# Wionerlol/MultimodalEmotionRecognition

Hardware: AMD Instinct MI355X
Metric: 3s-clip train steps/sec (B=32, xattn fusion) at 1/2/4/8 MI355X (higher is better)
Workload: dtype bf16; 1 GPU; ResNet18 + WavLM-base (frozen) + xattn fusion train step (fwd+bwd+Adam); per_gpu_batch=32, global_batch=32, frames=8, image=112, audio_samples=48000, parallelism=dp1

## Files before the change

### multimodalemotionrecognition_amd/csrc/conv.hip

```cpp
#include <type_traits>

#include "common.h"
#include "mer.h"

typedef __attribute__((ext_vector_type(4))) uint32_t u32x4;
typedef __attribute__((ext_vector_type(4))) short s16x4;

#ifdef MER_CONV_TIMING
static __device__ long long mer_ct_buf[512 * 64];
#define CT(k) \
  do { \
    if (threadIdx.x == 0 && blockIdx.x < 512 && (k) < 64) mer_ct_buf[blockIdx.x * 64 + (k)] = wall_clock64(); \
  } while (0)
MER_API int mer_ct_reset() {
  static long long zeros[512 * 64];
  return (int)hipMemcpyToSymbol(HIP_SYMBOL(mer_ct_buf), zeros, sizeof(zeros), 0, hipMemcpyHostToDevice);
}
MER_API int mer_ct_read(long long* host) {
  return (int)hipMemcpyFromSymbol(host, HIP_SYMBOL(mer_ct_buf), sizeof(long long) * 512 * 64, 0, hipMemcpyDeviceToHost);
}
static __device__ long long mer_ctp_buf[4096 * 8];
#define CTP(k) \
  do { \
    const unsigned b_ = blockIdx.y * gridDim.x + blockIdx.x; \
// ... 297 lines not shown
    for (int j = 0; j < JT; ++j) acc[i][j] = f32x4{0.f, 0.f, 0.f, 0.f};

  const int nk = (p_end - p_beg + 63) / 64;
  auto compute = [&](int cur) {
    const bf16_t* Aimg = &lds[cur][0];
    const bf16_t* Bimg = &lds[cur][64 * LDM];
#pragma unroll
    for (int s = 0; s < 2; ++s) {
      bf16x8 af[IT], bfr[JT];
#pragma unroll
      for (int i = 0; i < IT; ++i) af[i] = tr_frag(Aimg, LDM, s * 32, wm + i * 16);
#pragma unroll
      for (int j = 0; j < JT; ++j) bfr[j] = tr_frag(Bimg, LDN, s * 32, wn + j * 16);
#pragma unroll
      for (int i = 0; i < IT; ++i)
#pragma unroll
        for (int j = 0; j < JT; ++j) acc[i][j] = __builtin_amdgcn_mfma_f32_16x16x32_bf16(af[i], bfr[j], acc[i][j], 0, 0, 0);
    }
  };
  if (PF == 1) {
    if (nk > 0) {
      gload(ra, rb, okm, p_beg);
      lstore(0, ra, rb, okm);
    }
    __syncthreads();
    for (int kt = 0; kt < nk; ++kt) {
      const int cur = kt & 1;
      gload(ra, rb, okm, p_beg + (kt + 1 < nk ? kt + 1 : kt) * 64);
      compute(cur);
      if (kt + 1 < nk) lstore(cur ^ 1, ra, rb, okm);
      __syncthreads();
    }
  } else {
    auto kstep = [&](int k) { return p_beg + (k < nk ? k : nk - 1) * 64; };
    if (nk > 0) {
      gload(ra, rb, okm, p_beg);
      gload(ra2, rb2, okm2, kstep(1));
      lstore(0, ra, rb, okm);
    }
    lds_barrier();
    for (int kt = 0; kt < nk; kt += 2) {
      gload(ra, rb, okm, kstep(kt + 2));
      compute(0);
      if (kt + 1 < nk) lstore(1, ra2, rb2, okm2);
      lds_barrier();
      if (kt + 1 >= nk) break;
      gload(ra2, rb2, okm2, kstep(kt + 3));
      compute(1);
      if (kt + 2 < nk) lstore(0, ra, rb, okm);
      lds_barrier();
    }
  }
  float* slab = g.ws + (long)blockIdx.z * g.K * Ntot;
#pragma unroll
  for (int i = 0; i < IT; ++i)
#pragma unroll
    for (int j = 0; j < JT; ++j) {
      const int nn = n0 + wn + j * 16 + (lane & 15);
      if (nn >= Ntot) continue;
#pragma unroll
      for (int rr = 0; rr < 4; ++rr) {
        const int k = m0 + wm + i * 16 + (lane >> 4) * 4 + rr;
        if (k < g.K) slab[(long)k * Ntot + nn] = acc[i][j][rr];
      }
    }
}

__device__ __attribute__((aligned(16))) uint32_t mer_conv_zero16[4] = {0u, 0u, 0u, 0u};

__device__ __forceinline__ int wswz(int row, int nchunks) { return ((row & 7) << 1) & (nchunks - 1); }

template <int BM_, int BN_, int WM, int WN, int STAGES, int KS = 64, int KG = 1>
__global__ __launch_bounds__(64 * WM * WN * KG, KG > 1 ? WM * WN * KG / 4 : 2) void wgrad_pipe_kernel(WgradGeom g) {
  constexpr int WAVES = WM * WN;
  constexpr int ACW = BM_ / 8, BCW = BN_ / 8;
  constexpr int ARI = 64 / ACW, BRI = 64 / BCW;
  constexpr int IA = KS / ARI / WAVES, IB = KS / BRI / WAVES;
  static_assert(IA * ARI * WAVES == KS && IB * BRI * WAVES == KS, "the K-step must split into whole glds rows");
  static_assert(KS % 32 == 0, "MFMA k = 32 pixels");
  constexpr int IT = BM_ / WM / 16, JT = BN_ / WN / 16;
  constexpr int BUF = KS * (BM_ + BN_);
  extern __shared__ __attribute__((aligned(16))) bf16_t smem_all[];
  const int t = threadIdx.x, lane = t & 63, kg = (t >> 6) / WAVES, w = (t >> 6) % WAVES;
  bf16_t* const smem = smem_all + kg * STAGES * BUF;
  const int Ntot = g.R * g.S * g.C;
  const int P = g.N * g.Ho * g.Wo;
  const int wnx = (Ntot + BN_ - 1) / BN_, wny = (g.K + BM_ - 1) / BM_;
  int wtx, wty, zs;
  if (g.flat) {
    int tile;
    xcd_tile(blockIdx.x, wnx * wny, (int)gridDim.x, tile, zs);
    wty = tile / wnx;
    wtx = tile - wty * wnx;
  } else {
    xcd_tile(blockIdx.x, wnx, wnx * wny, wtx, wty);
    zs = blockIdx.z;
  }
  const int m0 = wty * BM_, n0 = wtx * BN_;
  const int p_beg = zs * g.pix_per_split, p_end = min(P, p_beg + g.pix_per_split);
  const int wm = (w / WN) * (BM_ / WM), wn = (w % WN) * (BN_ / WN);
  const bf16_t* zero = reinterpret_cast<const bf16_t*>(mer_conv_zero16);

  int arow[IA], acol[IA];
  bool acok[IA];
#pragma unroll
  for (int j = 0; j < IA; ++j) {
    const int row = (w * IA + j) * ARI + lane / ACW;
    arow[j] = row;
    acol[j] = m0 + ((lane % ACW) ^ wswz(row, ACW)) * 8;
    acok[j] = acol[j] < g.K;
  }
  int brow[IB], bc[IB], br[IB], bs[IB];
  bool bcok[IB];
  const float inv_C = 1.f / g.C, inv_S = 1.f / g.S, inv_HoWo = 1.f / (g.Ho * g.Wo), inv_Wo = 1.f / g.Wo;
#pragma unroll
  for (int j = 0; j < IB; ++j) {
    const int row = (w * IB + j) * BRI + lane / BCW;
    brow[j] = row;
    const int col = n0 + ((lane % BCW) ^ wswz(row, BCW)) * 8;
    bcok[j] = col < Ntot;
    const int cc = bcok[j] ? col : 0;
    const int tap = fdiv(cc, inv_C);
    bc[j] = cc - tap * g.C;
    br[j] = fdiv(tap, inv_S);
    bs[j] = tap - br[j] * g.S;
  }
  const int HoWo = g.Ho * g.Wo;
  auto stage = [&](int slot, int p0) {
    bf16_t* la = smem + slot * BUF;
    bf16_t* lb = la + KS * BM_;
#pragma unroll
    for (int j = 0; j < IA; ++j) {
      const int p = p0 + arow[j];
      glds16(p < p_end && acok[j] ? g.dY + (long)p * g.ldy + acol[j] : zero, la + (w * IA + j) * 512);
    }
#pragma unroll
    for (int j = 0; j < IB; ++j) {
      const int p = p0 + brow[j];
      const int pc = p < p_end ? p : p_beg;
      const int n = fdiv(pc, inv_HoWo);
      const int rem = pc - n * HoWo;
      const int oh = fdiv(rem, inv_Wo), ow = rem - oh * g.Wo;
      const int ih = oh * g.st - g.pad + br[j], iw = ow * g.st - g.pad + bs[j];
      const bool ok = p < p_end && bcok[j] && ih >= 0 && ih < g.H && iw >= 0 && iw < g.W;
      glds16(ok ? g.X + (((long)n * g.H + ih) * g.W + iw) * g.C + bc[j] : zero, lb + (w * IB + j) * 512);
    }
  };
  auto tr_frag = [&](const bf16_t* img, int CW, int k0, int c0) -> bf16x8 {
    const int q = (lane & 15) >> 2, p4 = (lane & 3) * 4;
    const int kr = k0 + 8 * (lane >> 4);
    const int lc = (c0 + p4) >> 3, sub = (c0 + p4) & 7;
    typedef __attribute__((address_space(3))) s16x4 lds_s16x4;
    const int r0 = kr + q, r1 = kr + 4 + q;
    const s16x4 lo = __builtin_amdgcn_ds_read_tr16_b64_v4i16(
        (lds_s16x4*)(img + r0 * CW * 8 + ((lc ^ wswz(r0, CW)) << 3) + sub));
    const s16x4 hi = __builtin_amdgcn_ds_read_tr16_b64_v4i16(
        (lds_s16x4*)(img + r1 * CW * 8 + ((lc ^ wswz(r1, CW)) << 3) + sub));
    typedef __attribute__((ext_vector_type(8))) short s16x8;
    s16x8 v = {lo[0], lo[1], lo[2], lo[3], hi[0], hi[1], hi[2], hi[3]};
    return __builtin_bit_cast(bf16x8, v);
  };

  f32x4 acc[IT][JT];
#pragma unroll
  for (int i = 0; i < IT; ++i)
#pragma unroll
    for (int j = 0; j < JT; ++j) acc[i][j] = f32x4{0.f, 0.f, 0.f, 0.f};
  const int nk_all = (p_end - p_beg + KS - 1) / KS;
  const int nkg = (nk_all + KG - 1) / KG, kb = kg * nkg;
  const int nk = nk_all - kb < nkg ? (nk_all - kb > 0 ? nk_all - kb : 0) : nkg;
  const int pk0 = p_beg + kb * KS;
  constexpr int G = IA + IB;
#pragma unroll
  for (int s = 0; s < STAGES - 1; ++s)
    if (s < nk) stage(s, pk0 + s * KS);
  for (int kt = 0; kt < nkg; ++kt) {
    const int left = nk - 1 - kt;
    const int ahead = left < (STAGES - 2) ? left : (STAGES - 2);
    wait_tiles_in_flight<G>(ahead);
    lds_barrier();
    if (kt + STAGES - 1 < nk) stage((kt + STAGES - 1) % STAGES, pk0 + (kt + STAGES - 1) * KS);
    if (KG > 1 && kt >= nk) continue;
    const bf16_t* Aimg = smem + (kt % STAGES) * BUF;
    const bf16_t* Bimg = Aimg + KS * BM_;
#pragma unroll
    for (int s = 0; s < KS / 32; ++s) {
      bf16x8 af[IT], bfr[JT];
#pragma unroll
      for (int i = 0; i < IT; ++i) af[i] = tr_frag(Aimg, ACW, s * 32, wm + i * 16);
#pragma unroll
      for (int j = 0; j < JT; ++j) bfr[j] = tr_frag(Bimg, BCW, s * 32, wn + j * 16);
      __builtin_amdgcn_s_setprio(1);
#pragma unroll
      for (int i = 0; i < IT; ++i)
#pragma unroll
        for (int j = 0; j < JT; ++j) acc[i][j] = __builtin_amdgcn_mfma_f32_16x16x32_bf16(af[i], bfr[j], acc[i][j], 0, 0, 0);
      __builtin_amdgcn_s_setprio(0);
    }
  }
  if constexpr (KG > 1) {
    constexpr int LDR = BN_ + 4;
    __syncthreads();
    float* const part = reinterpret_cast<float*>(smem_all);
    if (kg > 0) {
      float* mine = part + (kg - 1) * BM_ * LDR;
#pragma unroll
      for (int i = 0; i < IT; ++i)
#pragma unroll
        for (int j = 0; j < JT; ++j)
#pragma unroll
          for (int rr = 0; rr < 4; ++rr)
            mine[(wm + i * 16 + (lane >> 4) * 4 + rr) * LDR + wn + j * 16 + (lane & 15)] = acc[i][j][rr];
    }
    lds_barrier();
    if (kg > 0) return;
#pragma unroll
    for (int i = 0; i < IT; ++i)
#pragma unroll
      for (int j = 0; j < JT; ++j)
#pragma unroll
        for (int rr = 0; rr < 4; ++rr)
#pragma unroll
          for (int q = 1; q < KG; ++q)
            acc[i][j][rr] += part[(q - 1) * BM_ * LDR + (wm + i * 16 + (lane >> 4) * 4 + rr) * LDR + wn + j * 16 +
                                  (lane & 15)];
  }
  float* slab = g.ws + (long)zs * g.K * Ntot;
#pragma unroll
  for (int i = 0; i < IT; ++i)
#pragma unroll
    for (int j = 0; j < JT; ++j) {
      const int nn = n0 + wn + j * 16 + (lane & 15);
      if (nn >= Ntot) continue;
#pragma unroll
      for (int rr = 0; rr < 4; ++rr) {
        const int k = m0 + wm + i * 16 + (lane >> 4) * 4 + rr;
        if (k < g.K) slab[(long)k * Ntot + nn] = acc[i][j][rr];
      }
    }
}

template <int BM_, int BN_, int WM, int WN, int STAGES, int KS = 64, int KG = 1>
void launch_wgrad_pipe(const WgradGeom& g0, dim3 grid, hipStream_t st) {
  const size_t ring = (size_t)KG * STAGES * KS * (BM_ + BN_) * sizeof(bf16_t);
  const size_t xchg = (size_t)(KG - 1) * BM_ * (BN_ + 4) * sizeof(float);
  const size_t lds = ring > xchg ? ring : xchg;
  if (hipFuncSetAttribute(reinterpret_cast<const void*>(&wgrad_pipe_kernel<BM_, BN_, WM, WN, STAGES, KS, KG>),
                          hipFuncAttributeMaxDynamicSharedMemorySize, (int)lds) != hipSuccess)
    return;
  WgradGeom g = g0;
  g.flat = 1;
  const dim3 gr(grid.x * grid.z, 1, 1);
  hipLaunchKernelGGL((wgrad_pipe_kernel<BM_, BN_, WM, WN, STAGES, KS, KG>), gr, dim3(64 * WM * WN * KG), lds, st, g);
}

__global__ __launch_bounds__(256) void wgrad_reduce_kernel(int K, int C, int Creal, int RS, int splits, int SG,
                                                           float* __restrict__ ws) {
  __shared__ float part[256];
  const int E = 256 / SG, e = threadIdx.x % E, sg = threadIdx.x / E;
  const long total = (long)K * RS * C;
  const long idx = (long)blockIdx.x * E + e;
  float a0 = 0.f, a1 = 0.f, a2 = 0.f, a3 = 0.f;
  if (idx < total) {
    int z = sg;
    for (; z + 3 * SG < splits; z += 4 * SG) {
      a0 += ws[(long)z * total + idx];
      a1 += ws[(long)(z + SG) * total + idx];
      a2 += ws[(long)(z + 2 * SG) * total + idx];
      a3 += ws[(long)(z + 3 * SG) * total + idx];
    }
    for (; z < splits; z += SG) a0 += ws[(long)z * total + idx];
  }
  part[threadIdx.x] = (a0 + a1) + (a2 + a3);
  __syncthreads();
  if (sg != 0 || idx >= total) return;
  float s = 0.f;
  for (int q = 0; q < SG; ++q) s += part[q * E + e];
  ws[idx] = s;
}

__global__ __launch_bounds__(256) void wgrad_fold_scatter_kernel(int K, int C, int Creal, int RS, int splits,
                                                                 const float* __restrict__ ws, float* __restrict__ dw) {
  __shared__ float tile[49 * 32];
  const int k = blockIdx.y, c0 = blockIdx.x * 32;
  const long slab = (long)K * RS * C;
  const float* src = ws + (long)k * RS * C;
  for (int i = threadIdx.x; i < RS * 32; i += 256) {
    const int tap = i >> 5, c = c0 + (i & 31);
    const float* e = src + tap * C + (c < Creal ? c : 0);
    float s = 0.f;
    for (int z0 = 0; z0 < splits; z0 += 8) {
      float v[8];
#pragma unroll
      for (int q = 0; q < 8; ++q) v[q] = e[(long)(z0 + q < splits ? z0 + q : splits - 1) * slab];
#pragma unroll
      for (int q = 0; q < 8; ++q) s += z0 + q < splits ? v[q] : 0.f;
    }
    tile[i] = c < Creal ? s : 0.f;
  }
  __syncthreads();
  const int ncl = min(32, Creal - c0);
  const float inv_RS = 1.f / RS;
  float* dst = dw + ((long)k * Creal + c0) * RS;
  for (int i = threadIdx.x; i < ncl * RS; i += 256) {
    const int cl = fdiv(i, inv_RS), tap = i - cl * RS;
    dst[i] += tile[tap * 32 + cl];
  }
}

__global__ __launch_bounds__(256) void wgrad_scatter_kernel(int C, int Creal, int RS, const float* __restrict__ ws,
                                                            float* __restrict__ dw) {
  __shared__ float tile[49 * 32];
  const int k = blockIdx.y, c0 = blockIdx.x * 32;
  const float* src = ws + (long)k * RS * C;
  for (int i = threadIdx.x; i < RS * 32; i += 256) {
    const int tap = i >> 5, c = c0 + (i & 31);
    tile[i] = c < Creal ? src[tap * C + c] : 0.f;
  }
  __syncthreads();
  const int ncl = min(32, Creal - c0);
  const float inv_RS = 1.f / RS;
  float* dst = dw + ((long)k * Creal + c0) * RS;
// ... 480 lines not shown
    }
    flush();
    return;
  }
  conv_tile_stats<FM, FN, WM, WN>(g, acc, smemf, w, lane, m0, n0, M, stat_row);
  if (ct_slot >= 0) CT(ct_slot + 1);
  flush();
  if (ct_slot >= 0) CT(ct_slot + 2);
}

template <bool DGRAD, int FM, int FN, int WM, int WN, int WAVE_FLOATS, bool X2 = true>
__device__ __forceinline__ void conv_epilogue_acc_finish(const ConvGeom& g, EpiAcc<FN>& a, float* smemf, int w,
                                                         int lane, int n0, long row_id) {
  if constexpr (DGRAD) {
    if (!g.bnr_red) return;
    using E = EpiGeo<FM, FN, WAVE_FLOATS>;
    constexpr int TN = FN * 16, LPR = E::LPR;
    const int wr = w / WN, wc = w % WN;
    const int lc = (lane % LPR) * 8;
    const int colv = n0 + wc * TN + lc;
    const bool cok = colv < g.Ncols;
    const bool has_x2 = X2 && g.bnr_x2 != nullptr;
#pragma unroll
    for (int o = LPR; o < 64; o <<= 1)
#pragma unroll
      for (int e = 0; e < 8; ++e) {
        a.sA[e] += __shfl_xor(a.sA[e], o, 64);
        a.sB[e] += __shfl_xor(a.sB[e], o, 64);
        if (has_x2) a.sC[e] += __shfl_xor(a.sC[e], o, 64);
      }
    float* red = smemf;
    lds_barrier();
    if (wr > 0 && lane < LPR)
#pragma unroll
      for (int e = 0; e < 8; ++e) {
        float* o = red + ((wr * WN + wc) * TN + lc + e) * 3;
        o[0] = a.sA[e];
        o[1] = a.sB[e];
        o[2] = a.sC[e];
      }
    lds_barrier();
    if (wr != 0 || lane >= LPR || !cok) return;
#pragma unroll
    for (int e = 0; e < 8; ++e)
#pragma unroll
      for (int q = 1; q < WM; ++q) {
        const float* o = red + ((q * WN + wc) * TN + lc + e) * 3;
        a.sA[e] += o[0];
        a.sB[e] += o[1];
        a.sC[e] += o[2];
      }
    const long slab = row_id * g.Ncols * 2 + 2 * colv;
#pragma unroll
    for (int e = 0; e < 8; e += 2) {
      *reinterpret_cast<f32x4*>(g.bnr_red + slab + 2 * e) = f32x4{a.sA[e], a.sB[e], a.sA[e + 1], a.sB[e + 1]};
      if (g.bnr_red2)
        *reinterpret_cast<f32x4*>(g.bnr_red2 + slab + 2 * e) = f32x4{a.sA[e], a.sC[e], a.sA[e + 1], a.sC[e + 1]};
    }
  } else {
    if (!g.stats) return;
    conv_stats_finish<FN, WM, WN>(g, a.fs, smemf, w, lane, n0, row_id);
  }
}

constexpr int conv_pipe_wpe(int nw, int bm, int bn, int stages, bool dgrad, bool par, int lds_bytes = 0) {
  return (nw >= 16 || 2 * lds_bytes > 160 * 1024)
             ? (nw >= 4 ? nw / 4 : 1)
             : nw == 8 ? ((dgrad && (bm == 256 || (!par && bm == 128 && bn == 128 && stages == 3))) ? 2 : 4) : 2;
}
constexpr int conv_pipe_lds(int bm, int bn, int stages, int ks, int kg) {
  return kg * stages * (bm + bn) * ks * 2 > (kg > 1 ? kg * bm * (bn + 4) * 4 : 0)
             ? kg * stages * (bm + bn) * ks * 2
             : kg * bm * (bn + 4) * 4;
}

template <int BM_, int BN_, int NW>
struct KgLayout {
  static constexpr int WM = (NW >= 4 && BM_ / 4 >= 16) ? 4 : (NW >= 2 ? 2 : 1);
  static constexpr int WN = NW / WM;
  static_assert(WM * WN == NW && BM_ % (16 * WM) == 0 && BN_ % (16 * WN) == 0, "split-K epilogue layout");
};

template <bool DGRAD, bool PAR, int BM_, int BN_, int WM = 2, int WN = 2, int STAGES = 2, int KS = 64, bool X2 = true,
          int KG = 1>
__global__ __launch_bounds__(64 * WM * WN * KG, conv_pipe_wpe(WM * WN * KG, BM_, BN_, STAGES, DGRAD, PAR,
                                                              conv_pipe_lds(BM_, BN_, STAGES, KS, KG))) void conv_pipe_kernel(ConvGeom g) {
  constexpr int WAVES = WM * WN;
  constexpr int CW = KS / 8, RPG = 64 / CW;
  constexpr int IA = BM_ / RPG / WAVES, IB = BN_ / RPG / WAVES;
  static_assert(IA * RPG * WAVES == BM_ && IB * RPG * WAVES == BN_, "tile rows must split into whole glds pieces");
  static_assert(KS == 64 || KS == 32, "K-tile");
  static_assert(KG == 1 || KG == 2 || KG == 4, "K-groups");
  constexpr int TM = BM_ / WM, TN = BN_ / WN, FM = TM / 16, FN = TN / 16;
  constexpr int BUF = (BM_ + BN_) * KS;
  extern __shared__ __attribute__((aligned(16))) bf16_t smem_all[];
  const int t = threadIdx.x, lane = t & 63, kg = (t >> 6) / WAVES, w = (t >> 6) % WAVES;
  bf16_t* const smem = smem_all + kg * STAGES * BUF;
  ParClass pc{};
  int M, Kr, rowsH, rowsW;
  int Kr0 = 0;
  if (PAR) {
    pc = par_class(g, par_cls());
    M = g.N * pc.Hc * pc.Wc;
    Kr0 = pc.nr * pc.ns * g.IC;
    Kr = Kr0 + ((g.X2 && pc.ph == 0 && pc.pw == 0) ? g.K2 : 0);
    rowsH = pc.Hc;
    rowsW = pc.Wc;
  } else {
    M = g.N * g.OH * g.OW;
    Kr = g.Kred;
    rowsH = g.OH;
    rowsW = g.OW;
  }
  const int nx = (g.Ncols + BN_ - 1) / BN_, ny = (M + BM_ - 1) / BM_;
  if ((int)blockIdx.x >= nx * ny) return;
  CTP(0);
  int tx, ty;
  xcd_tile(blockIdx.x, nx, nx * ny, tx, ty);
  const int m0 = ty * BM_, n0 = tx * BN_;
  const int wr = w / WN, wc = w % WN;

  int an[IA], aoh[IA], aow[IA], acl[IA];
  bool aok[IA];
#pragma unroll
  for (int j = 0; j < IA; ++j) {
    const int r = (w * IA + j) * RPG + lane / CW;
    const int m = m0 + r;
    aok[j] = m < M;
    const int mm = aok[j] ? m : 0;
    an[j] = mm / (rowsH * rowsW);
    const int rem = mm - an[j] * rowsH * rowsW;
    aoh[j] = rem / rowsW;
    aow[j] = rem - aoh[j] * rowsW;
    acl[j] = cswz_k<CW>(r, lane % CW) * 8;
  }
  const bf16_t* pb[IB];
  const bf16_t* pb2[IB];
  int bcl[IB];
  bool bok[IB];
#pragma unroll
  for (int j = 0; j < IB; ++j) {
    const int r = (w * IB + j) * RPG + lane / CW;
    const int n = n0 + r;
    bok[j] = n < g.Ncols;
    pb[j] = g.Wt + (long)(bok[j] ? n : 0) * g.Kred;
    pb2[j] = g.Wt2 + (long)(bok[j] ? n : 0) * g.K2;
    bcl[j] = cswz_k<CW>(r, lane % CW) * 8;
  }
  const float inv_IC = 1.f / g.IC, inv_S = 1.f / g.S, inv_ns = PAR ? 1.f / pc.ns : 1.f;
  const bf16_t* zero = reinterpret_cast<const bf16_t*>(mer_conv_zero16);
  auto par_a_src = [&](int n, int hh, int ww, bool rowok, int kk) -> const bf16_t* {
    if (!rowok || kk >= Kr) return zero;
    if (kk >= Kr0)
      return g.X2 + (((long)n * g.IH + hh) * g.IW + ww) * g.K2 + (kk - Kr0);
    const int tap = fdiv(kk, inv_IC), c = kk - tap * g.IC;
    const int ri = fdiv(tap, inv_ns), si = tap - ri * pc.ns;
    const int ih = hh + pc.dh0 - ri, iw = ww + pc.dw0 - si;
    if (ih < 0 || ih >= g.IH || iw < 0 || iw >= g.IW) return zero;
    return g.X + (((long)n * g.IH + ih) * g.IW + iw) * g.IC + c;
  };
  auto par_b_off = [&](int kk) -> int {
    const int tap = fdiv(kk, inv_IC), c = kk - tap * g.IC;
    const int ri = fdiv(tap, inv_ns), si = tap - ri * pc.ns;
    return ((pc.r0 + 2 * ri) * g.S + pc.s0 + 2 * si) * g.IC + c;
  };
  auto stage = [&](int buf, int k0) {
    bf16_t* la = smem + buf * BUF;
    bf16_t* lb = la + BM_ * KS;
#pragma unroll
    for (int j = 0; j < IA; ++j) {
      const bf16_t* src = PAR ? par_a_src(an[j], aoh[j], aow[j], aok[j], k0 + acl[j])
                              : conv_a_src<DGRAD>(g, an[j], aoh[j], aow[j], aok[j], k0 + acl[j], inv_IC, inv_S);
      glds16(src, la + (w * IA + j) * 512);
    }
#pragma unroll
    for (int j = 0; j < IB; ++j) {
      const int kk = k0 + bcl[j];
      const bool ok = bok[j] && kk < Kr;
      const bf16_t* src = !PAR ? pb[j] + kk : (kk >= Kr0 ? pb2[j] + (kk - Kr0) : pb[j] + par_b_off(kk));
      glds16(ok ? src : zero, lb + (w * IB + j) * 512);
    }
  };

  f32x4 acc[FM][FN];
#pragma unroll
  for (int i = 0; i < FM; ++i)
#pragma unroll
    for (int j = 0; j < FN; ++j) acc[i][j] = f32x4{0.f, 0.f, 0.f, 0.f};

  const int fr = lane & 15, fq = lane >> 4;
  const int nk_all = (Kr + KS - 1) / KS;
  const int nkg = (nk_all + KG - 1) / KG, kb = kg * nkg;
  const int nk = nk_all - kb < nkg ? (nk_all - kb > 0 ? nk_all - kb : 0) : nkg;
  const int kofs = kb * KS;
  constexpr int G = IA + IB;
  static_assert(STAGES >= 2 && STAGES <= 4, "ring depth");
#pragma unroll
  for (int p = 0; p < STAGES - 1; ++p)
    if (p < nk) stage(p, kofs + p * KS);
  CTP(1);
  for (int kt = 0; kt < nkg; ++kt) {
    const int left = nk - 1 - kt;
    const int ahead = left < (STAGES - 2) ? left : (STAGES - 2);
    wait_tiles_in_flight<G>(ahead);
    lds_barrier();
    if (kt + STAGES - 1 < nk) stage((kt + STAGES - 1) % STAGES, kofs + (kt + STAGES - 1) * KS);
    if (KG > 1 && kt >= nk) continue;
    const bf16_t* la = smem + (kt % STAGES) * BUF;
    const bf16_t* lb = la + BM_ * KS;
#pragma unroll
    for (int s = 0; s < KS / 32; ++s) {
      bf16x8 af[FM], bfr[FN];
#pragma unroll
      for (int i = 0; i < FM; ++i) {
        const int r = wr * TM + i * 16 + fr;
        af[i] = *reinterpret_cast<const bf16x8*>(la + r * KS + cswz_k<CW>(r, s * 4 + fq) * 8);
      }
#pragma unroll
      for (int j = 0; j < FN; ++j) {
        const int r = wc * TN + j * 16 + fr;
        bfr[j] = *reinterpret_cast<const bf16x8*>(lb + r * KS + cswz_k<CW>(r, s * 4 + fq) * 8);
      }
      __builtin_amdgcn_s_setprio(1);
#pragma unroll
      for (int i = 0; i < FM; ++i)
#pragma unroll
        for (int j = 0; j < FN; ++j) acc[i][j] = __builtin_amdgcn_mfma_f32_16x16x32_bf16(af[i], bfr[j], acc[i][j], 0, 0, 0);
      __builtin_amdgcn_s_setprio(0);
    }
  }
  CTP(2);

  auto out_row = [&](int row) -> long {
    if (!PAR) return (long)row;
    const int n = row / (pc.Hc * pc.Wc);
    const int rem = row - n * pc.Hc * pc.Wc;
    const int hh = rem / pc.Wc, ww = rem - hh * pc.Wc;
    return ((long)n * g.OH + 2 * hh + pc.ph) * g.OW + 2 * ww + pc.pw;
  };
  auto red_row = [&]() -> long {
    long row_id = ty;
    if (PAR)
      for (int c2 = 0; c2 < par_cls(); ++c2) {
        const ParClass q = par_class(g, c2);
        row_id += (g.N * q.Hc * q.Wc + BM_ - 1) / BM_;
      }
    return row_id;
  };
  constexpr int EWF = STAGES * BUF / 2 / WAVES;
  const int ct_slot = 10;
  if constexpr (KG > 1) {
    using L = KgLayout<BM_, BN_, WAVES * KG>;
    constexpr int LDR = BN_ + 4;
    constexpr int TM2 = BM_ / L::WM, TN2 = BN_ / L::WN, FM2 = TM2 / 16, FN2 = TN2 / 16;
    using E2 = EpiGeo<FM2, FN2, EWF>;
    const int w2 = t >> 6, wr2 = w2 / L::WN, wc2 = w2 % L::WN;
    constexpr bool PF = DGRAD && E2::NP == 1;
    EpiPre<E2::NP> pre;
    if constexpr (PF)
      conv_epilogue_prefetch<DGRAD, FM2, FN2, L::WM, L::WN, EWF, decltype(out_row), E2::NP, X2>(g, pre, w2, lane, m0,
                                                                                                n0, M, out_row);
    __syncthreads();
    float* const part = reinterpret_cast<float*>(smem_all);
    {
      float* mine = part + kg * BM_ * LDR;
#pragma unroll
      for (int i = 0; i < FM; ++i)
#pragma unroll
        for (int j = 0; j < FN; ++j)
#pragma unroll
          for (int r = 0; r < 4; ++r) mine[(wr * TM + i * 16 + fq * 4 + r) * LDR + wc * TN + j * 16 + fr] = acc[i][j][r];
    }
    lds_barrier();
    f32x4 acc2[FM2][FN2];
#pragma unroll
    for (int i = 0; i < FM2; ++i)
#pragma unroll
      for (int j = 0; j < FN2; ++j)
#pragma unroll
        for (int r = 0; r < 4; ++r) {
          const int e = (wr2 * TM2 + i * 16 + fq * 4 + r) * LDR + wc2 * TN2 + j * 16 + fr;
          float s = part[e];
#pragma unroll
          for (int q = 1; q < KG; ++q) s += part[q * BM_ * LDR + e];
          acc2[i][j][r] = s;
        }
    lds_barrier();
    CTP(3);
    if constexpr (PF)
      conv_epilogue_vec<DGRAD, FM2, FN2, L::WM, L::WN, EWF, decltype(out_row), decltype(pre), false, X2>(
          g, acc2, reinterpret_cast<float*>(smem_all), w2, lane, m0, n0, M, g.bnr_red ? red_row() : 0l, ty, out_row,
          &pre, ct_slot);
    else
      conv_epilogue_vec<DGRAD, FM2, FN2, L::WM, L::WN, EWF, decltype(out_row), EpiNone, false, X2>(
          g, acc2, reinterpret_cast<float*>(smem_all), w2, lane, m0, n0, M, (DGRAD && g.bnr_red) ? red_row() : 0l, ty,
          out_row, static_cast<const EpiNone*>(nullptr), ct_slot);
    CTP(4);
    return;
  }
  if (g.vec) {
    using E1 = EpiGeo<FM, FN, EWF>;
    if constexpr (DGRAD && E1::NP == 1) {
      EpiPre<E1::NP> pre;
      conv_epilogue_prefetch<DGRAD, FM, FN, WM, WN, EWF, decltype(out_row), E1::NP, X2>(g, pre, w, lane, m0, n0, M,
                                                                                         out_row);
      __syncthreads();
      CTP(3);
      conv_epilogue_vec<DGRAD, FM, FN, WM, WN, EWF, decltype(out_row), decltype(pre), false, X2>(
          g, acc, reinterpret_cast<float*>(smem), w, lane, m0, n0, M, g.bnr_red ? red_row() : 0l, ty, out_row, &pre,
          ct_slot);
    } else {
      __syncthreads();
// ... 30 lines not shown
  if (DGRAD && g.bnr_red) {
    float ps[FN][3];
#pragma unroll
    for (int j = 0; j < FN; ++j) {
      const int col = n0 + wc * TN + j * 16 + fr;
      const bool cok = col < g.Ncols;
      const float mu = cok ? g.bnr_ms[2 * col] : 0.f, rs = cok ? g.bnr_ms[2 * col + 1] : 0.f;
      const float mu2 = (cok && g.bnr_x2) ? g.bnr_ms2[2 * col] : 0.f;
      const float rs2 = (cok && g.bnr_x2) ? g.bnr_ms2[2 * col + 1] : 0.f;
      float s1 = 0.f, s2 = 0.f, s3 = 0.f;
#pragma unroll
      for (int i = 0; i < FM; ++i)
#pragma unroll
        for (int r = 0; r < 4; ++r) {
          const int row = m0 + wr * TM + i * 16 + fq * 4 + r;
          if (row < M && cok) {
            const long e = out_row(row) * g.ldy + col;
            const float gv = bf2f(g.bnr_mask[e]) > 0.f ? acc[i][j][r] : 0.f;
            s1 += gv;
            s2 += gv * (bf2f(g.bnr_x[e]) - mu) * rs;
            if (g.bnr_x2) s3 += gv * (bf2f(g.bnr_x2[e]) - mu2) * rs2;
          }
        }
#pragma unroll
      for (int o = 16; o < 64; o <<= 1) {
        s1 += __shfl_xor(s1, o, 64);
        s2 += __shfl_xor(s2, o, 64);
        s3 += __shfl_xor(s3, o, 64);
      }
      ps[j][0] = s1;
      ps[j][1] = s2;
      ps[j][2] = s3;
    }
    float* red = reinterpret_cast<float*>(smem);
    __syncthreads();
    if (wr > 0 && fq == 0)
#pragma unroll
      for (int j = 0; j < FN; ++j)
#pragma unroll
        for (int q = 0; q < 3; ++q) red[((wr * WN + wc) * FN * 16 + j * 16 + fr) * 3 + q] = ps[j][q];
    __syncthreads();
    if (wr == 0 && fq == 0) {
      long row_id = ty;
      if (PAR)
        for (int c2 = 0; c2 < par_cls(); ++c2) {
          const ParClass q = par_class(g, c2);
          row_id += (g.N * q.Hc * q.Wc + BM_ - 1) / BM_;
        }
      const long slab = row_id * g.Ncols * 2;
#pragma unroll
      for (int j = 0; j < FN; ++j) {
        const int col = n0 + wc * TN + j * 16 + fr;
        float t0 = ps[j][0], t1 = ps[j][1], t2 = ps[j][2];
#pragma unroll
        for (int q = 1; q < WM; ++q) {
          const float* o = red + ((q * WN + wc) * FN * 16 + j * 16 + fr) * 3;
          t0 += o[0];
          t1 += o[1];
          t2 += o[2];
        }
        if (col < g.Ncols) {
          g.bnr_red[slab + 2 * col] = t0;
          g.bnr_red[slab + 2 * col + 1] = t1;
          if (g.bnr_red2) {
            g.bnr_red2[slab + 2 * col] = t0;
            g.bnr_red2[slab + 2 * col + 1] = t2;
          }
        }
      }
    }
  }
  }
  if (g.stats) conv_tile_stats<FM, FN, WM, WN>(g, acc, reinterpret_cast<float*>(smem), w, lane, m0, n0, M, ty);
}

template <bool DGRAD, bool PAR, int BM_, int BN_, int WM = 2, int WN = 2, int STAGES = 2, int KS = 64, int KG = 1>
int launch_conv_pipe_t(ConvGeom& g, hipStream_t st) {
  const int Mg = PAR ? g.N * ((g.OH + 1) / 2) * ((g.OW + 1) / 2) : g.N * g.OH * g.OW;
  const long tiles = (long)((Mg + BM_ - 1) / BM_) * ((g.Ncols + BN_ - 1) / BN_);
  const size_t ring = (size_t)KG * STAGES * (BM_ + BN_) * KS * sizeof(bf16_t);
  const size_t kgred = KG > 1 ? (size_t)KG * BM_ * (BN_ + 4) * sizeof(float) : 0;
  const size_t lds = ring > kgred ? ring : kgred;
  if (KG > 1 && !g.vec) return (int)hipErrorInvalidValue;
  if constexpr (DGRAD && !PAR) {
    if (!g.bnr_x2) {
      if (hipFuncSetAttribute(
              reinterpret_cast<const void*>(&conv_pipe_kernel<DGRAD, PAR, BM_, BN_, WM, WN, STAGES, KS, false, KG>),
              hipFuncAttributeMaxDynamicSharedMemorySize, (int)lds) != hipSuccess)
        return (int)hipErrorInvalidConfiguration;
      hipLaunchKernelGGL((conv_pipe_kernel<DGRAD, PAR, BM_, BN_, WM, WN, STAGES, KS, false, KG>),
                         dim3((unsigned)tiles, 1), dim3(64 * WM * WN * KG), lds, st, g);
      return (int)hipGetLastError();
    }
  }
  if (hipFuncSetAttribute(
          reinterpret_cast<const void*>(&conv_pipe_kernel<DGRAD, PAR, BM_, BN_, WM, WN, STAGES, KS, true, KG>),
          hipFuncAttributeMaxDynamicSharedMemorySize, (int)lds) != hipSuccess)
    return (int)hipErrorInvalidConfiguration;
  hipLaunchKernelGGL((conv_pipe_kernel<DGRAD, PAR, BM_, BN_, WM, WN, STAGES, KS, true, KG>),
                     dim3((unsigned)tiles, PAR ? 4 : 1), dim3(64 * WM * WN * KG), lds, st, g);
  return (int)hipGetLastError();
}

template <bool DGRAD, bool PAR>
int launch_conv_pipe(ConvGeom& g, hipStream_t st, int variant) {
  const int M = PAR ? g.N * g.OH * g.OW / 4 : g.N * g.OH * g.OW;
  const int bn = g.Ncols <= 64 ? 64 : 128;
  const long tiles128 = (long)((M + 127) / 128) * ((g.Ncols + bn - 1) / bn) * (PAR ? 4 : 1);
  const bool small_m = tiles128 < 384;
  if (variant == 7) {
    if (bn == 64)
      return PAR ? launch_conv_pipe_t<DGRAD, PAR, 64, 64, 2, 2, 2, 64, 2>(g, st)
                 : launch_conv_pipe_t<DGRAD, PAR, 64, 64, 2, 2, 3, 64, 2>(g, st);
    return PAR ? launch_conv_pipe_t<DGRAD, PAR, 64, 128, 2, 4, 2, 64, 2>(g, st)
               : launch_conv_pipe_t<DGRAD, PAR, 64, 128, 2, 4, 3, 64, 2>(g, st);
  }
  if (variant == 3 && !small_m) {
    if constexpr (DGRAD) {
      return launch_conv_pipe_t<DGRAD, PAR, 256, 64, 4, 2>(g, st);
    } else {
      if (bn == 64) return launch_conv_pipe_t<DGRAD, PAR, 256, 64, 4, 2>(g, st);
      return launch_conv_pipe_t<DGRAD, PAR, 256, 128, 4, 4>(g, st);
    }
  }
  if (variant == 5) {
    if (bn == 64)
      return small_m ? launch_conv_pipe_t<DGRAD, PAR, 64, 64, 2, 2, 4, 32>(g, st)
                     : launch_conv_pipe_t<DGRAD, PAR, 128, 64, 2, 2, 4, 32>(g, st);
    return small_m ? launch_conv_pipe_t<DGRAD, PAR, 64, 128, 2, 2, 4, 32>(g, st)
                   : launch_conv_pipe_t<DGRAD, PAR, 128, 128, 2, 4, 4, 32>(g, st);
  }
  if (variant == 4) {
    if (bn == 64)
      return small_m ? launch_conv_pipe_t<DGRAD, PAR, 64, 64, 2, 2, 3>(g, st)
                     : launch_conv_pipe_t<DGRAD, PAR, 128, 64, 4, 2, 3>(g, st);
    return small_m ? launch_conv_pipe_t<DGRAD, PAR, 64, 128, 2, 4, 3>(g, st)
                   : launch_conv_pipe_t<DGRAD, PAR, 128, 128, 2, 4, 3>(g, st);
  }
  if (variant >= 2) {
    if (bn == 64)
      return small_m ? (PAR ? launch_conv_pipe_t<DGRAD, PAR, 64, 64, 2, 2>(g, st)
                            : launch_conv_pipe_t<DGRAD, PAR, 64, 64, 2, 2, 3>(g, st))
                     : launch_conv_pipe_t<DGRAD, PAR, 128, 64, 4, 2>(g, st);
    return small_m ? (PAR ? launch_conv_pipe_t<DGRAD, PAR, 64, 128, 2, 4>(g, st)
                          : launch_conv_pipe_t<DGRAD, PAR, 64, 128, 2, 4, 3>(g, st))
                   : launch_conv_pipe_t<DGRAD, PAR, 128, 128, 2, 4>(g, st);
  }
  if (bn == 64)
    return small_m ? launch_conv_pipe_t<DGRAD, PAR, 64, 64>(g, st) : launch_conv_pipe_t<DGRAD, PAR, 128, 64>(g, st);
  return small_m ? launch_conv_pipe_t<DGRAD, PAR, 64, 128>(g, st) : launch_conv_pipe_t<DGRAD, PAR, 128, 128>(g, st);
}

template <bool DGRAD>
int launch_conv(ConvGeom& g, hipStream_t st) {
  const int M = g.N * g.OH * g.OW;
  const int bn = g.Ncols <= 64 ? 64 : 128;
  const long tiles128 = (long)((M + 127) / 128) * ((g.Ncols + bn - 1) / bn);
  const bool small_m = tiles128 < 384;
  const int nx = (g.Ncols + bn - 1) / bn;
  if (bn == 64) {
    if (small_m) {
      hipLaunchKernelGGL((conv_kernel<DGRAD, 64, 64>), dim3(nx * ((M + 63) / 64)), dim3(256), 0, st, g);
    } else {
      hipLaunchKernelGGL((conv_kernel<DGRAD, 128, 64>), dim3(nx * ((M + 127) / 128)), dim3(256), 0, st, g);
    }
  } else {
    if (small_m) {
      hipLaunchKernelGGL((conv_kernel<DGRAD, 64, 128>), dim3(nx * ((M + 63) / 64)), dim3(256), 0, st, g);
    } else {
      hipLaunchKernelGGL((conv_kernel<DGRAD, 128, 128>), dim3(nx * ((M + 127) / 128)), dim3(256), 0, st, g);
    }
  }
  return (int)hipGetLastError();
}

namespace halo {
constexpr int BM = 128;
template <int C_, int R_, int PAD_, int W_, int IHX_>
struct Geo {
  static constexpr int C = C_, R = R_, PAD = PAD_, W = W_, IHX = IHX_;
  static constexpr int KRED = R * R * C, WCH = KRED / 8;
  static constexpr int CPP = C / 8;
  static constexpr int HW = W + R - 1;
  static constexpr int ROWS = (W + BM - 2) / W + 1 + (R - 1) + IHX;
// ... 1535 lines not shown
```

Measured before the change: 211.6 steps/s.

## Replace per-stage im2col index division with incremental pointer stepping in conv kernels

The wgrad kernel now computes the per-lane source pointers and output coordinates once, then advances them by a fixed step with wrap corrections each K-stage. This replaces the per-stage float-reciprocal divisions for n/oh/ow. The forward and dgrad conv_pipe kernel gains a FAST template path, selected when IC is a multiple of KS and the filter has at most 32 taps. That path precomputes a per-row tap-validity bitmask and walks taps incrementally instead of decoding each k index. The goal is to cut scalar and vector address arithmetic in the load stage, at the cost of more live registers and another kernel instantiation.

New measurement: 217.7 steps/s, median of 6. +2.9%, better.

```diff
diff --git a/multimodalemotionrecognition_amd/csrc/conv.hip b/multimodalemotionrecognition_amd/csrc/conv.hip
--- a/multimodalemotionrecognition_amd/csrc/conv.hip
+++ b/multimodalemotionrecognition_amd/csrc/conv.hip
@@ -403,6 +403,7 @@
   constexpr int BUF = KS * (BM_ + BN_);
   extern __shared__ __attribute__((aligned(16))) bf16_t smem_all[];
   const int t = threadIdx.x, lane = t & 63, kg = (t >> 6) / WAVES, w = (t >> 6) % WAVES;
+  CTP(0);
   bf16_t* const smem = smem_all + kg * STAGES * BUF;
   const int Ntot = g.R * g.S * g.C;
   const int P = g.N * g.Ho * g.Wo;
@@ -422,50 +423,73 @@
   const int wm = (w / WN) * (BM_ / WM), wn = (w % WN) * (BN_ / WN);
   const bf16_t* zero = reinterpret_cast<const bf16_t*>(mer_conv_zero16);
 
-  int arow[IA], acol[IA];
+  const int nk_all = (p_end - p_beg + KS - 1) / KS;
+  const int nkg = (nk_all + KG - 1) / KG, kb = __builtin_amdgcn_readfirstlane(kg * nkg);
+  const int nk = nk_all - kb < nkg ? (nk_all - kb > 0 ? nk_all - kb : 0) : nkg;
+  const int pk0 = p_beg + kb * KS;
+
+  const int HoWo = g.Ho * g.Wo;
+  const bf16_t* ap[IA];
+  int arow[IA];
   bool acok[IA];
 #pragma unroll
   for (int j = 0; j < IA; ++j) {
-    const int row = (w * IA + j) * ARI + lane / ACW;
-    arow[j] = row;
-    acol[j] = m0 + ((lane % ACW) ^ wswz(row, ACW)) * 8;
-    acok[j] = acol[j] < g.K;
-  }
-  int brow[IB], bc[IB], br[IB], bs[IB];
+    arow[j] = (w * IA + j) * ARI + lane / ACW;
+    const int acol = m0 + ((lane % ACW) ^ wswz(arow[j], ACW)) * 8;
+    acok[j] = acol < g.K;
+    ap[j] = g.dY + ((long)(pk0 + arow[j]) * g.ldy + acol);
+  }
+  const long a_step = (long)KS * g.ldy;
+  const bf16_t* bp[IB];
+  int brow[IB], boh[IB], bow[IB], bdr[IB], bds[IB];
   bool bcok[IB];
-  const float inv_C = 1.f / g.C, inv_S = 1.f / g.S, inv_HoWo = 1.f / (g.Ho * g.Wo), inv_Wo = 1.f / g.Wo;
 #pragma unroll
   for (int j = 0; j < IB; ++j) {
-    const int row = (w * IB + j) * BRI + lane / BCW;
-    brow[j] = row;
-    const int col = n0 + ((lane % BCW) ^ wswz(row, BCW)) * 8;
+    brow[j] = (w * IB + j) * BRI + lane / BCW;
+    const int col = n0 + ((lane % BCW) ^ wswz(brow[j], BCW)) * 8;
     bcok[j] = col < Ntot;
     const int cc = bcok[j] ? col : 0;
-    const int tap = fdiv(cc, inv_C);
-    bc[j] = cc - tap * g.C;
-    br[j] = fdiv(tap, inv_S);
-    bs[j] = tap - br[j] * g.S;
-  }
-  const int HoWo = g.Ho * g.Wo;
-  auto stage = [&](int slot, int p0) {
+    const int tap = cc / g.C, c = cc - tap * g.C;
+    const int r = tap / g.S;
+    bdr[j] = r - g.pad;
+    bds[j] = tap - r * g.S - g.pad;
+    const int p = pk0 + brow[j];
+    const int n = p / HoWo, rem = p - n * HoWo;
+    boh[j] = rem / g.Wo;
+    bow[j] = rem - boh[j] * g.Wo;
+    bp[j] = g.X + ((((long)n * g.H + boh[j] * g.st + bdr[j]) * g.W + bow[j] * g.st + bds[j]) * g.C + c);
+  }
+  const int s_dn = KS / HoWo, s_rem = KS - s_dn * HoWo, s_dh = s_rem / g.Wo, s_dw = s_rem - s_dh * g.Wo;
+  const int d_step = ((s_dn * g.H + s_dh * g.st) * g.W + s_dw * g.st) * g.C;
+  const int d_wrap_w = g.st * (g.W - g.Wo) * g.C;
+  const int d_wrap_h = (g.H - g.Ho * g.st) * g.W * g.C;
+  int p_left = p_end - pk0;
+  auto stage = [&](int slot) {
     bf16_t* la = smem + slot * BUF;
     bf16_t* lb = la + KS * BM_;
 #pragma unroll
     for (int j = 0; j < IA; ++j) {
-      const int p = p0 + arow[j];
-      glds16(p < p_end && acok[j] ? g.dY + (long)p * g.ldy + acol[j] : zero, la + (w * IA + j) * 512);
+      glds16(((int)(arow[j] < p_left) & (int)acok[j]) ? ap[j] : zero, la + (w * IA + j) * 512);
+      ap[j] += a_step;
     }
 #pragma unroll
     for (int j = 0; j < IB; ++j) {
-      const int p = p0 + brow[j];
-      const int pc = p < p_end ? p : p_beg;
-      const int n = fdiv(pc, inv_HoWo);
-      const int rem = pc - n * HoWo;
-      const int oh = fdiv(rem, inv_Wo), ow = rem - oh * g.Wo;
-      const int ih = oh * g.st - g.pad + br[j], iw = ow * g.st - g.pad + bs[j];
-      const bool ok = p < p_end && bcok[j] && ih >= 0 && ih < g.H && iw >= 0 && iw < g.W;
-      glds16(ok ? g.X + (((long)n * g.H + ih) * g.W + iw) * g.C + bc[j] : zero, lb + (w * IB + j) * 512);
-    }
+      const int ok = (int)(brow[j] < p_left) & (int)bcok[j] &
+                     (int)((unsigned)(__mul24(boh[j], g.st) + bdr[j]) < (unsigned)g.H) &
+                     (int)((unsigned)(__mul24(bow[j], g.st) + bds[j]) < (unsigned)g.W);
+      glds16(ok ? bp[j] : zero, lb + (w * IB + j) * 512);
+      int d = d_step;
+      bow[j] += s_dw;
+      const bool cw = bow[j] >= g.Wo;
+      bow[j] -= cw ? g.Wo : 0;
+      d += cw ? d_wrap_w : 0;
+      boh[j] += s_dh + (cw ? 1 : 0);
+      const bool ch = boh[j] >= g.Ho;
+      boh[j] -= ch ? g.Ho : 0;
+      d += ch ? d_wrap_h : 0;
+      bp[j] += d;
+    }
+    p_left -= KS;
   };
   auto tr_frag = [&](const bf16_t* img, int CW, int k0, int c0) -> bf16x8 {
     const int q = (lane & 15) >> 2, p4 = (lane & 3) * 4;
@@ -487,22 +511,22 @@
   for (int i = 0; i < IT; ++i)
 #pragma unroll
     for (int j = 0; j < JT; ++j) acc[i][j] = f32x4{0.f, 0.f, 0.f, 0.f};
-  const int nk_all = (p_end - p_beg + KS - 1) / KS;
-  const int nkg = (nk_all + KG - 1) / KG, kb = kg * nkg;
-  const int nk = nk_all - kb < nkg ? (nk_all - kb > 0 ? nk_all - kb : 0) : nkg;
-  const int pk0 = p_beg + kb * KS;
   constexpr int G = IA + IB;
 #pragma unroll
   for (int s = 0; s < STAGES - 1; ++s)
-    if (s < nk) stage(s, pk0 + s * KS);
+    if (s < nk) stage(s);
+  int wslot = STAGES - 1, rslot = 0;
+  CTP(1);
   for (int kt = 0; kt < nkg; ++kt) {
     const int left = nk - 1 - kt;
     const int ahead = left < (STAGES - 2) ? left : (STAGES - 2);
     wait_tiles_in_flight<G>(ahead);
     lds_barrier();
-    if (kt + STAGES - 1 < nk) stage((kt + STAGES - 1) % STAGES, pk0 + (kt + STAGES - 1) * KS);
+    if (kt + STAGES - 1 < nk) stage(wslot);
+    wslot = wslot == STAGES - 1 ? 0 : wslot + 1;
+    const bf16_t* Aimg = smem + rslot * BUF;
+    rslot = rslot == STAGES - 1 ? 0 : rslot + 1;
     if (KG > 1 && kt >= nk) continue;
-    const bf16_t* Aimg = smem + (kt % STAGES) * BUF;
     const bf16_t* Bimg = Aimg + KS * BM_;
 #pragma unroll
     for (int s = 0; s < KS / 32; ++s) {
@@ -519,6 +543,7 @@
       __builtin_amdgcn_s_setprio(0);
     }
   }
+  CTP(2);
   if constexpr (KG > 1) {
     constexpr int LDR = BN_ + 4;
     __syncthreads();
@@ -546,6 +571,7 @@
             acc[i][j][rr] += part[(q - 1) * BM_ * LDR + (wm + i * 16 + (lane >> 4) * 4 + rr) * LDR + wn + j * 16 +
                                   (lane & 15)];
   }
+  CTP(3);
   float* slab = g.ws + (long)zs * g.K * Ntot;
 #pragma unroll
   for (int i = 0; i < IT; ++i)
@@ -559,6 +585,7 @@
         if (k < g.K) slab[(long)k * Ntot + nn] = acc[i][j][rr];
       }
     }
+  CTP(4);
 }
 
 template <int BM_, int BN_, int WM, int WN, int STAGES, int KS = 64, int KG = 1>
@@ -1205,7 +1232,7 @@
 };
 
 template <bool DGRAD, bool PAR, int BM_, int BN_, int WM = 2, int WN = 2, int STAGES = 2, int KS = 64, bool X2 = true,
-          int KG = 1>
+          int KG = 1, bool FAST = false>
 __global__ __launch_bounds__(64 * WM * WN * KG, conv_pipe_wpe(WM * WN * KG, BM_, BN_, STAGES, DGRAD, PAR,
                                                               conv_pipe_lds(BM_, BN_, STAGES, KS, KG))) void conv_pipe_kernel(ConvGeom g) {
   constexpr int WAVES = WM * WN;
@@ -1243,67 +1270,29 @@
   const int m0 = ty * BM_, n0 = tx * BN_;
   const int wr = w / WN, wc = w % WN;
 
-  int an[IA], aoh[IA], aow[IA], acl[IA];
-  bool aok[IA];
-#pragma unroll
-  for (int j = 0; j < IA; ++j) {
-    const int r = (w * IA + j) * RPG + lane / CW;
-    const int m = m0 + r;
-    aok[j] = m < M;
-    const int mm = aok[j] ? m : 0;
-    an[j] = mm / (rowsH * rowsW);
-    const int rem = mm - an[j] * rowsH * rowsW;
-    aoh[j] = rem / rowsW;
-    aow[j] = rem - aoh[j] * rowsW;
-    acl[j] = cswz_k<CW>(r, lane % CW) * 8;
-  }
-  const bf16_t* pb[IB];
-  const bf16_t* pb2[IB];
-  int bcl[IB];
+  auto a_row = [&](int j, int& n, int& oh, int& ow, bool& ok) {
+    const int m = m0 + (w * IA + j) * RPG + lane / CW;
+    ok = m < M;
+    const int mm = ok ? m : 0;
+    n = mm / (rowsH * rowsW);
+    const int rem = mm - n * rowsH * rowsW;
+    oh = rem / rowsW;
+    ow = rem - oh * rowsW;
+  };
+  int acl[IA];
+#pragma unroll
+  for (int j = 0; j < IA; ++j) acl[j] = cswz_k<CW>((w * IA + j) * RPG + lane / CW, lane % CW) * 8;
+  int bcl[IB], bn[IB];
   bool bok[IB];
 #pragma unroll
   for (int j = 0; j < IB; ++j) {
     const int r = (w * IB + j) * RPG + lane / CW;
     const int n = n0 + r;
     bok[j] = n < g.Ncols;
-    pb[j] = g.Wt + (long)(bok[j] ? n : 0) * g.Kred;
-    pb2[j] = g.Wt2 + (long)(bok[j] ? n : 0) * g.K2;
+    bn[j] = bok[j] ? n : 0;
     bcl[j] = cswz_k<CW>(r, lane % CW) * 8;
   }
-  const float inv_IC = 1.f / g.IC, inv_S = 1.f / g.S, inv_ns = PAR ? 1.f / pc.ns : 1.f;
   const bf16_t* zero = reinterpret_cast<const bf16_t*>(mer_conv_zero16);
-  auto par_a_src = [&](int n, int hh, int ww, bool rowok, int kk) -> const bf16_t* {
-    if (!rowok || kk >= Kr) return zero;
-    if (kk >= Kr0)
-      return g.X2 + (((long)n * g.IH + hh) * g.IW + ww) * g.K2 + (kk - Kr0);
-    const int tap = fdiv(kk, inv_IC), c = kk - tap * g.IC;
-    const int ri = fdiv(tap, inv_ns), si = tap - ri * pc.ns;
-    const int ih = hh + pc.dh0 - ri, iw = ww + pc.dw0 - si;
-    if (ih < 0 || ih >= g.IH || iw < 0 || iw >= g.IW) return zero;
-    return g.X + (((long)n * g.IH + ih) * g.IW + iw) * g.IC + c;
-  };
-  auto par_b_off = [&](int kk) -> int {
-    const int tap = fdiv(kk, inv_IC), c = kk - tap * g.IC;
-    const int ri = fdiv(tap, inv_ns), si = tap - ri * pc.ns;
-    return ((pc.r0 + 2 * ri) * g.S + pc.s0 + 2 * si) * g.IC + c;
-  };
-  auto stage = [&](int buf, int k0) {
-    bf16_t* la = smem + buf * BUF;
-    bf16_t* lb = la + BM_ * KS;
-#pragma unroll
-    for (int j = 0; j < IA; ++j) {
-      const bf16_t* src = PAR ? par_a_src(an[j], aoh[j], aow[j], aok[j], k0 + acl[j])
-                              : conv_a_src<DGRAD>(g, an[j], aoh[j], aow[j], aok[j], k0 + acl[j], inv_IC, inv_S);
-      glds16(src, la + (w * IA + j) * 512);
-    }
-#pragma unroll
-    for (int j = 0; j < IB; ++j) {
-      const int kk = k0 + bcl[j];
-      const bool ok = bok[j] && kk < Kr;
-      const bf16_t* src = !PAR ? pb[j] + kk : (kk >= Kr0 ? pb2[j] + (kk - Kr0) : pb[j] + par_b_off(kk));
-      glds16(ok ? src : zero, lb + (w * IB + j) * 512);
-    }
-  };
 
   f32x4 acc[FM][FN];
 #pragma unroll
@@ -1313,44 +1302,175 @@
 
   const int fr = lane & 15, fq = lane >> 4;
   const int nk_all = (Kr + KS - 1) / KS;
-  const int nkg = (nk_all + KG - 1) / KG, kb = kg * nkg;
+  const int nkg = (nk_all + KG - 1) / KG, kb = __builtin_amdgcn_readfirstlane(kg * nkg);
   const int nk = nk_all - kb < nkg ? (nk_all - kb > 0 ? nk_all - kb : 0) : nkg;
   const int kofs = kb * KS;
   constexpr int G = IA + IB;
   static_assert(STAGES >= 2 && STAGES <= 4, "ring depth");
-#pragma unroll
-  for (int p = 0; p < STAGES - 1; ++p)
-    if (p < nk) stage(p, kofs + p * KS);
-  CTP(1);
-  for (int kt = 0; kt < nkg; ++kt) {
-    const int left = nk - 1 - kt;
-    const int ahead = left < (STAGES - 2) ? left : (STAGES - 2);
-    wait_tiles_in_flight<G>(ahead);
-    lds_barrier();
-    if (kt + STAGES - 1 < nk) stage((kt + STAGES - 1) % STAGES, kofs + (kt + STAGES - 1) * KS);
-    if (KG > 1 && kt >= nk) continue;
-    const bf16_t* la = smem + (kt % STAGES) * BUF;
-    const bf16_t* lb = la + BM_ * KS;
-#pragma unroll
-    for (int s = 0; s < KS / 32; ++s) {
-      bf16x8 af[FM], bfr[FN];
-#pragma unroll
-      for (int i = 0; i < FM; ++i) {
-        const int r = wr * TM + i * 16 + fr;
-        af[i] = *reinterpret_cast<const bf16x8*>(la + r * KS + cswz_k<CW>(r, s * 4 + fq) * 8);
-      }
-#pragma unroll
-      for (int j = 0; j < FN; ++j) {
-        const int r = wc * TN + j * 16 + fr;
-        bfr[j] = *reinterpret_cast<const bf16x8*>(lb + r * KS + cswz_k<CW>(r, s * 4 + fq) * 8);
-      }
-      __builtin_amdgcn_s_setprio(1);
-#pragma unroll
-      for (int i = 0; i < FM; ++i)
-#pragma unroll
-        for (int j = 0; j < FN; ++j) acc[i][j] = __builtin_amdgcn_mfma_f32_16x16x32_bf16(af[i], bfr[j], acc[i][j], 0, 0, 0);
-      __builtin_amdgcn_s_setprio(0);
-    }
+  auto k_loop = [&](auto&& stage) {
+#pragma unroll
+    for (int p = 0; p < STAGES - 1; ++p)
+      if (p < nk) stage(p);
+    int wslot = STAGES - 1, rslot = 0;
+    CTP(1);
+    for (int kt = 0; kt < nkg; ++kt) {
+      const int left = nk - 1 - kt;
+      const int ahead = left < (STAGES - 2) ? left : (STAGES - 2);
+      wait_tiles_in_flight<G>(ahead);
+      lds_barrier();
+      if (kt + STAGES - 1 < nk) stage(wslot);
+      wslot = wslot == STAGES - 1 ? 0 : wslot + 1;
+      const bf16_t* la = smem + rslot * BUF;
+      rslot = rslot == STAGES - 1 ? 0 : rslot + 1;
+      if (KG > 1 && kt >= nk) continue;
+      const bf16_t* lb = la + BM_ * KS;
+#pragma unroll
+      for (int s = 0; s < KS / 32; ++s) {
+        bf16x8 af[FM], bfr[FN];
+#pragma unroll
+        for (int i = 0; i < FM; ++i) {
+          const int r = wr * TM + i * 16 + fr;
+          af[i] = *reinterpret_cast<const bf16x8*>(la + r * KS + cswz_k<CW>(r, s * 4 + fq) * 8);
+        }
+#pragma unroll
+        for (int j = 0; j < FN; ++j) {
+          const int r = wc * TN + j * 16 + fr;
+          bfr[j] = *reinterpret_cast<const bf16x8*>(lb + r * KS + cswz_k<CW>(r, s * 4 + fq) * 8);
+        }
+        __builtin_amdgcn_s_setprio(1);
+#pragma unroll
+        for (int i = 0; i < FM; ++i)
+#pragma unroll
+          for (int j = 0; j < FN; ++j)
+            acc[i][j] = __builtin_amdgcn_mfma_f32_16x16x32_bf16(af[i], bfr[j], acc[i][j], 0, 0, 0);
+        __builtin_amdgcn_s_setprio(0);
+      }
+    }
+  };
+
+  if constexpr (FAST) {
+    const bool has_ds = PAR && Kr > Kr0;
+    constexpr bool NEG = DGRAD || PAR;
+    const int nr = PAR ? pc.nr : g.R, ns = PAR ? pc.ns : g.S;
+    const bf16_t* fa[IA];
+    unsigned fm[IA];
+#pragma unroll
+    for (int j = 0; j < IA; ++j) {
+      int n, oh, ow;
+      bool ok;
+      a_row(j, n, oh, ow, ok);
+      const int h0 = PAR ? oh + pc.dh0 : DGRAD ? oh + g.pad : oh * g.st - g.pad;
+      const int w0 = PAR ? ow + pc.dw0 : DGRAD ? ow + g.pad : ow * g.st - g.pad;
+      unsigned cm = 0, m = 0;
+      for (int si = 0; si < ns; ++si) cm |= (unsigned)((unsigned)(NEG ? w0 - si : w0 + si) < (unsigned)g.IW) << si;
+      for (int ri = 0; ri < nr; ++ri)
+        if ((unsigned)(NEG ? h0 - ri : h0 + ri) < (unsigned)g.IH) m |= cm << (ri * ns);
+      fm[j] = ok ? m : 0u;
+      fa[j] = g.X + ((((long)n * g.IH + h0) * g.IW + w0) * g.IC + acl[j]);
+    }
+    const bf16_t* fb[IB];
+#pragma unroll
+    for (int j = 0; j < IB; ++j) fb[j] = g.Wt + ((long)bn[j] * g.Kred + bcl[j]);
+    int f_ic = g.IC, f_c, f_tap, f_ri, f_si, f_aoff, f_boff;
+    bool f_ds = false;
+    auto tap_offsets = [&]() {
+      const int ao = (f_ri * g.IW + f_si) * g.IC;
+      f_aoff = NEG ? -ao : ao;
+      f_boff = PAR ? ((pc.r0 + 2 * f_ri) * g.S + pc.s0 + 2 * f_si) * g.IC : f_tap * g.IC;
+    };
+    auto enter_ds = [&]() {
+      f_ds = true;
+      f_ic = g.K2;
+      f_c = f_tap = f_ri = f_si = f_aoff = f_boff = 0;
+#pragma unroll
+      for (int j = 0; j < IA; ++j) {
+        int n, hh, ww;
+        bool ok;
+        a_row(j, n, hh, ww, ok);
+        fm[j] = ok ? 1u : 0u;
+        fa[j] = g.X2 + ((((long)n * g.IH + hh) * g.IW + ww) * g.K2 + acl[j]);
+      }
+#pragma unroll
+      for (int j = 0; j < IB; ++j) fb[j] = g.Wt2 + ((long)bn[j] * g.K2 + bcl[j]);
+    };
+    if (has_ds && kofs >= Kr0) {
+      enter_ds();
+      f_c = kofs - Kr0;
+    } else {
+      f_tap = kofs / g.IC;
+      f_c = kofs - f_tap * g.IC;
+      f_ri = f_tap / (ns > 0 ? ns : 1);
+      f_si = f_tap - f_ri * ns;
+      tap_offsets();
+    }
+    k_loop([&](int buf) {
+      bf16_t* la = smem + buf * BUF;
+      bf16_t* lb = la + BM_ * KS;
+      const unsigned tbit = 1u << (f_tap & 31);
+      const long ao = f_aoff + f_c, bo = f_boff + f_c;
+#pragma unroll
+      for (int j = 0; j < IA; ++j) glds16((fm[j] & tbit) ? fa[j] + ao : zero, la + (w * IA + j) * 512);
+#pragma unroll
+      for (int j = 0; j < IB; ++j) glds16(bok[j] ? fb[j] + bo : zero, lb + (w * IB + j) * 512);
+      f_c += KS;
+      if (f_c == f_ic) {
+        f_c = 0;
+        ++f_tap;
+        if (++f_si == ns) {
+          f_si = 0;
+          ++f_ri;
+        }
+        tap_offsets();
+        if (has_ds && !f_ds && f_tap == nr * ns) enter_ds();
+      }
+    });
+  } else {
+    int an[IA], aoh[IA], aow[IA];
+    bool aok[IA];
+#pragma unroll
+    for (int j = 0; j < IA; ++j) a_row(j, an[j], aoh[j], aow[j], aok[j]);
+    const bf16_t* pb[IB];
+    const bf16_t* pb2[IB];
+#pragma unroll
+    for (int j = 0; j < IB; ++j) {
+      pb[j] = g.Wt + (long)bn[j] * g.Kred;
+      pb2[j] = g.Wt2 + (long)bn[j] * g.K2;
+    }
+    const float inv_IC = 1.f / g.IC, inv_S = 1.f / g.S, inv_ns = PAR ? 1.f / pc.ns : 1.f;
+    auto par_a_src = [&](int n, int hh, int ww, bool rowok, int kk) -> const bf16_t* {
+      if (!rowok || kk >= Kr) return zero;
+      if (kk >= Kr0)
+        return g.X2 + (((long)n * g.IH + hh) * g.IW + ww) * g.K2 + (kk - Kr0);
+      const int tap = fdiv(kk, inv_IC), c = kk - tap * g.IC;
+      const int ri = fdiv(tap, inv_ns), si = tap - ri * pc.ns;
+      const int ih = hh + pc.dh0 - ri, iw = ww + pc.dw0 - si;
+      if (ih < 0 || ih >= g.IH || iw < 0 || iw >= g.IW) return zero;
+      return g.X + (((long)n * g.IH + ih) * g.IW + iw) * g.IC + c;
+    };
+    auto par_b_off = [&](int kk) -> int {
+      const int tap = fdiv(kk, inv_IC), c = kk - tap * g.IC;
+      const int ri = fdiv(tap, inv_ns), si = tap - ri * pc.ns;
+      return ((pc.r0 + 2 * ri) * g.S + pc.s0 + 2 * si) * g.IC + c;
+    };
+    int k0 = kofs;
+    k_loop([&](int buf) {
+      bf16_t* la = smem + buf * BUF;
+      bf16_t* lb = la + BM_ * KS;
+#pragma unroll
+      for (int j = 0; j < IA; ++j) {
+        const bf16_t* src = PAR ? par_a_src(an[j], aoh[j], aow[j], aok[j], k0 + acl[j])
+                                : conv_a_src<DGRAD>(g, an[j], aoh[j], aow[j], aok[j], k0 + acl[j], inv_IC, inv_S);
+        glds16(src, la + (w * IA + j) * 512);
+      }
+#pragma unroll
+      for (int j = 0; j < IB; ++j) {
+        const int kk = k0 + bcl[j];
+        const bool ok = bok[j] && kk < Kr;
+        const bf16_t* src = !PAR ? pb[j] + kk : (kk >= Kr0 ? pb2[j] + (kk - Kr0) : pb[j] + par_b_off(kk));
+        glds16(ok ? src : zero, lb + (w * IB + j) * 512);
+      }
+      k0 += KS;
+    });
   }
   CTP(2);
 
@@ -1547,24 +1667,22 @@
   const size_t kgred = KG > 1 ? (size_t)KG * BM_ * (BN_ + 4) * sizeof(float) : 0;
   const size_t lds = ring > kgred ? ring : kgred;
   if (KG > 1 && !g.vec) return (int)hipErrorInvalidValue;
+  const bool fast = PAR ? (g.IC % KS == 0 && (!g.X2 || g.K2 % KS == 0) && ((g.R + 1) / 2) * ((g.S + 1) / 2) <= 32)
+                        : (g.IC % KS == 0 && g.R * g.S <= 32 && (!DGRAD || g.st == 1));
+  auto launch = [&](void (*kern)(ConvGeom), unsigned gy) -> int {
+    if (hipFuncSetAttribute(reinterpret_cast<const void*>(kern), hipFuncAttributeMaxDynamicSharedMemorySize,
+                            (int)lds) != hipSuccess)
+      return (int)hipErrorInvalidConfiguration;
+    hipLaunchKernelGGL(kern, dim3((unsigned)tiles, gy), dim3(64 * WM * WN * KG), lds, st, g);
+    return (int)hipGetLastError();
+  };
   if constexpr (DGRAD && !PAR) {
-    if (!g.bnr_x2) {
-      if (hipFuncSetAttribute(
-              reinterpret_cast<const void*>(&conv_pipe_kernel<DGRAD, PAR, BM_, BN_, WM, WN, STAGES, KS, false, KG>),
-              hipFuncAttributeMaxDynamicSharedMemorySize, (int)lds) != hipSuccess)
-        return (int)hipErrorInvalidConfiguration;
-      hipLaunchKernelGGL((conv_pipe_kernel<DGRAD, PAR, BM_, BN_, WM, WN, STAGES, KS, false, KG>),
-                         dim3((unsigned)tiles, 1), dim3(64 * WM * WN * KG), lds, st, g);
-      return (int)hipGetLastError();
-    }
-  }
-  if (hipFuncSetAttribute(
-          reinterpret_cast<const void*>(&conv_pipe_kernel<DGRAD, PAR, BM_, BN_, WM, WN, STAGES, KS, true, KG>),
-          hipFuncAttributeMaxDynamicSharedMemorySize, (int)lds) != hipSuccess)
-    return (int)hipErrorInvalidConfiguration;
-  hipLaunchKernelGGL((conv_pipe_kernel<DGRAD, PAR, BM_, BN_, WM, WN, STAGES, KS, true, KG>),
-                     dim3((unsigned)tiles, PAR ? 4 : 1), dim3(64 * WM * WN * KG), lds, st, g);
-  return (int)hipGetLastError();
+    if (!g.bnr_x2)
+      return fast ? launch(&conv_pipe_kernel<DGRAD, PAR, BM_, BN_, WM, WN, STAGES, KS, false, KG, true>, 1)
+                  : launch(&conv_pipe_kernel<DGRAD, PAR, BM_, BN_, WM, WN, STAGES, KS, false, KG, false>, 1);
+  }
+  return fast ? launch(&conv_pipe_kernel<DGRAD, PAR, BM_, BN_, WM, WN, STAGES, KS, true, KG, true>, PAR ? 4 : 1)
+              : launch(&conv_pipe_kernel<DGRAD, PAR, BM_, BN_, WM, WN, STAGES, KS, true, KG, false>, PAR ? 4 : 1);
 }
 
 template <bool DGRAD, bool PAR>
```
